# sourmash-bio/sourmash

Measured on AMD Instinct MI355X. Metric: Gbase/s sketched (k=31, scaled=1000), higher is better.
Workload: dtype u64; 1 GPU; C2: sketch synthetic random DNA resident in HBM as ASCII, per GPU 1000 records of 10000000 bases (10000000000 bases, 10000001000 bytes with their separators), k=31 scaled=1000 seed=42; one step = k-mer kernel + radix sort + unique; records_per_gpu=1000, record_len=10000000, bases_per_gpu=10000000000, bytes_per_gpu=10000001000, ksize=31, scaled=1000, unique_hashes_rank0=9998668, unique_hashes_job=9998668, collectives=none (the exchange runs with --full)

## Files before the change

sourmash_amd/csrc/capi_ingest.cpp:

```cpp
#include <stdio.h>
#include <algorithm>
#include <atomic>
#include <chrono>
#include "capi_common.hpp"
#include "ingest.hpp"
#include "pargz.hpp"
#include "residues.hpp"
#include "sigload.hpp"
#include "uniform_sort_core.hpp"

using namespace smg;

namespace {

static size_t sketch_ws_raw_bytes(uint64_t cap) { return al256(cap * 8); }
static size_t sketch_ws_sort_bytes(uint64_t cap, bool counts) {
    return std::max(sort_unique_temp_bytes(cap), sort_unique_uniform_temp_bound(cap, counts));
}

struct SortCounters { std::atomic<uint64_t> bucket{0}, small{0}, fellback{0}; };
static SortCounters& sort_counters() { static SortCounters c; return c; }

static void uniform_sort_and_report(const uint64_t* d_keys, const unsigned long long* d_n, uint64_t n_max, uint64_t thr, uint64_t* d_out,
                                    uint64_t* d_counts, uint64_t* d_n_out, void* d_head, void* d_tmp, size_t tmp_bytes, hipStream_t st,
                                    uint64_t report[3]) {
    uint64_t* d_report = (uint64_t*)d_head;
    uint32_t* d_flag = (uint32_t*)((char*)d_head + 64);
    hip_check(sort_unique_uniform(d_keys, d_n, n_max, thr, d_out, d_counts, d_n_out, d_flag, d_tmp, tmp_bytes, st), "sort_unique_uniform");
    hip_check(sort_report_launch(d_n, d_n_out, d_flag, d_report, st), "sort_report");
    hip_check(hipMemcpyAsync(report, d_report, 24, hipMemcpyDeviceToHost, st), "D2H");
    hip_check(hipStreamSynchronize(st), "sync");
}
static void count_sort_call(uint64_t n_max, uint64_t thr, size_t tmp_bytes, bool counts, bool fellback) {
    if (fellback) ++sort_counters().fellback;
    else if (sort_unique_uniform_form(n_max, thr, tmp_bytes, counts) == US_SMALL) ++sort_counters().small;
    else ++sort_counters().bucket;
}
static int key_bits(uint64_t thr) {
    int bits = 64;
    if (thr != ~0ull) { bits = 1; while (bits < 64 && (thr >> bits)) ++bits; }
    return bits;
}

}

extern "C" {

uint64_t smgpu_signature_add_file(SourmashSignature* p, const char* path, uint64_t* n_records) {
    return landing<uint64_t>([&]() -> uint64_t {
        if (!path) throw err_internal("null path");
        std::vector<KmerMinHash*> mhs;
// ... 107 lines not shown
}

uint64_t smgpu_sketch_dna_raw(const uint8_t* d_seq, uint64_t len, uint32_t ksize, uint64_t seed, uint64_t max_hash,
                              uint64_t* d_out, uint64_t cap, uint64_t* d_result, void* d_ws, uint64_t ws_bytes,
                              void* stream) {
    uint64_t ret = ~0ull;
    landing_void([&] {
        hipStream_t st = (hipStream_t)stream;
        if (ws_bytes < smgpu_sketch_workspace_bytes(cap)) throw err_internal("workspace too small (smgpu_sketch_workspace_bytes)");
        uint64_t* d_raw = (uint64_t*)d_ws;
        void* d_head = (char*)d_ws + sketch_ws_raw_bytes(cap);
        void* d_tmp = (char*)d_head + 256;
        const size_t tmp_bytes = (size_t)(ws_bytes - sketch_ws_raw_bytes(cap) - 256);
        const uint64_t thr = max_hash ? max_hash : ~0ull;
        check_dna_ksize(ksize);
        hip_check(hipMemsetAsync(d_result, 0, 16, st), "memset");
        hip_check(sketch_dna_launch(d_seq, len, ksize, seed, thr, d_raw, (unsigned long long*)d_result, cap, st), "sketch_dna");
        uint64_t report[3] = {0, 0, 0};
        uniform_sort_and_report(d_raw, (const unsigned long long*)d_result, cap, thr, d_out, nullptr, d_result + 1, d_head, d_tmp, tmp_bytes,
                                st, report);
        const uint64_t kept = report[0];
        if (kept > cap)
            throw err_internal("output capacity too small: " + std::to_string(kept) + " kept hashes > capacity " + std::to_string(cap));
        count_sort_call(cap, thr, tmp_bytes, false, report[2] != 0);
        if (report[2] == 0) { ret = report[1]; return; }
        hip_check(sort_unique(d_raw, kept, d_out, nullptr, d_result + 1, d_tmp, tmp_bytes, key_bits(thr), st), "sort_unique");
        unsigned long long nu = 0;
        hip_check(hipMemcpyAsync(&nu, d_result + 1, 8, hipMemcpyDeviceToHost, st), "D2H");
        hip_check(hipStreamSynchronize(st), "sync");
        ret = nu;
    });
    return ret;
}

uint64_t smgpu_sort_unique_uniform_workspace_bytes(uint64_t n_max, int32_t counts) {
// ... 141 lines not shown
```

sourmash_amd/csrc/device_api.hpp:

```cpp
#pragma once
#include <hip/hip_runtime.h>
#include <stdint.h>
#include <stddef.h>
#include "find_core.hpp"

namespace smg {

hipError_t sketch_dna_launch(const uint8_t* d_seq, uint64_t len, uint32_t k, uint64_t seed, uint64_t thr,
                             uint64_t* d_out, unsigned long long* d_count, uint64_t cap, hipStream_t stream);
hipError_t sketch_dna_launch_grid(const uint8_t* d_seq, uint64_t len, uint32_t k, uint64_t seed, uint64_t thr,
                                  uint64_t* d_out, unsigned long long* d_count, uint64_t cap, uint32_t grid, hipStream_t stream);
struct SketchMultiOut { uint64_t thr; uint64_t* out; unsigned long long* count; uint64_t cap; };
bool sketch_dna_multi_supported(const uint32_t* ks, int n);
hipError_t sketch_dna_multi_launch(const uint8_t* d_new, uint64_t n_new, const uint32_t* ks, int n, uint64_t seed, const SketchMultiOut* outs,
                                   hipStream_t stream);
hipError_t sketch_dna_words_launch(const uint8_t* d_seq, uint64_t len, uint32_t k, uint64_t seed, uint64_t thr, uint64_t* d_out,
                                   unsigned long long* d_count, uint64_t cap, bool dense, hipStream_t stream);
uint32_t sketch_dna_max_k();
hipError_t kmer_hashes_launch(const uint8_t* d_seq, uint64_t len, uint32_t k, uint64_t seed, uint64_t* d_out,
                              uint64_t n_kmers, hipStream_t stream);
hipError_t first_invalid_launch(const uint8_t* d_seq, uint64_t len, unsigned long long* d_first, hipStream_t stream);

hipError_t hll_dna_launch(const uint8_t* d_seq, uint64_t len, uint32_t k, uint32_t p, uint32_t* d_regs, hipStream_t stream);
hipError_t hll_hashes_launch(const uint64_t* d_hashes, uint64_t n, uint32_t p, uint32_t* d_regs, bool skip_zero, hipStream_t stream);
// ... 19 lines not shown
hipError_t residue_windows_launch(const uint8_t* d_aa, uint64_t n, uint32_t k, uint64_t seed, uint64_t thr, uint64_t* d_out,
                                  unsigned long long* d_count, uint64_t cap, bool dense, hipStream_t stream);

size_t sort_unique_temp_bytes(uint64_t n);
struct TagSegment { uint64_t src, dst, n; };
hipError_t tag_gather_launch(const uint64_t* d_src, const TagSegment* d_segs, uint32_t n_segs, uint64_t* d_dst, int hbits, hipStream_t stream);
hipError_t sort_unique(uint64_t* d_keys, uint64_t n, uint64_t* d_out, uint64_t* d_counts, uint64_t* d_n_out,
                       void* d_temp, size_t temp_bytes, int bits, hipStream_t stream);

hipError_t sort_unique_uniform(const uint64_t* d_keys, const unsigned long long* d_n, uint64_t n_max, uint64_t thr, uint64_t* d_out,
                               uint64_t* d_counts, uint64_t* d_n_out, uint32_t* d_fellback, void* d_temp, size_t temp_bytes,
                               hipStream_t stream);
size_t sort_unique_uniform_temp_bytes(uint64_t n_max, uint64_t thr, bool counts);
size_t sort_unique_uniform_temp_bound(uint64_t n_max, bool counts);
uint32_t sort_unique_uniform_form(uint64_t n_max, uint64_t thr, size_t temp_bytes, bool counts);
hipError_t sort_report_launch(const unsigned long long* d_n, const uint64_t* d_n_out, const uint32_t* d_fellback, uint64_t* d_report,
                              hipStream_t stream);

size_t sort_pairs_temp_bytes(uint64_t n);
hipError_t sort_pairs(const uint64_t* d_keys_in, uint64_t* d_keys_out, const uint64_t* d_vals_in, uint64_t* d_vals_out, uint64_t n,
                      int bits, void* d_temp, size_t temp_bytes, hipStream_t stream);
size_t rle_pairs_temp_bytes(uint64_t n);
hipError_t rle_pairs(const uint64_t* d_a, const uint64_t* d_b, uint64_t n, uint64_t* d_out_a, uint64_t* d_out_b, uint64_t* d_counts,
                     uint64_t* d_n_out, void* d_temp, size_t temp_bytes, hipStream_t stream);

hipError_t records_pairs_launch(const uint8_t* d_seq, uint64_t len, uint32_t k, uint64_t seed, uint64_t thr, uint64_t* d_hash,
                                uint64_t* d_pos, unsigned long long* d_count, uint64_t cap, hipStream_t stream);
hipError_t records_check_starts_launch(const uint64_t* d_starts, uint64_t n_records, uint64_t len, unsigned long long* d_bad,
                                       hipStream_t stream);
size_t records_csr_temp_bytes(uint64_t n_pairs);
// ... 106 lines not shown
```

sourmash_amd/csrc/kmer_core.hpp:

```cpp
#pragma once
#include "murmur3.hpp"
#include <utility>

namespace smg {

SMG_HD uint32_t perm_b32(uint32_t hi, uint32_t lo, uint32_t sel) {
#if defined(__HIP_DEVICE_COMPILE__)
    return __builtin_amdgcn_perm(hi, lo, sel);
#else
    const uint64_t v = ((uint64_t)hi << 32) | lo;
    uint32_t r = 0;
    for (int i = 0; i < 4; ++i) {
        const uint32_t s = (sel >> (8 * i)) & 0xff;
        uint32_t b;
        if (s < 8) b = (uint32_t)(v >> (8 * s)) & 0xff;
        else if (s == 0x0c) b = 0;
        else b = 0xff;
        r |= b << (8 * i);
    }
    return r;
#endif
}

SMG_HD uint32_t alignbyte_b32(uint32_t hi, uint32_t lo, uint32_t n) {
// ... 229 lines not shown
    process_window<K, P, EARLY, PLAIN, true, LATE>(U, C, dirty, seed, thr, static_cast<Emit&&>(emit), std::make_integer_sequence<int, P>{});
}


template <int K, int P, int BLOCK, int R = 1>
struct TileGeom {
    using G = LaneGeom<K, P>;
    static constexpr int WINDOW = BLOCK * P;
    static constexpr int TILE = R * WINDOW;
    static constexpr int LANE_RD = ((G::NW + 3) / 4) * 4;
    static constexpr int chunks(int rounds) { return ((rounds * BLOCK - 1) * (P / 4) + LANE_RD + 3) / 4; }
    static constexpr int IN_DW = (R * BLOCK - 1) * (P / 4) + LANE_RD;
    static constexpr int IN_CHUNKS = chunks(R);
};

SMG_HD uint32_t sk_tile_rounds(uint64_t thr, uint32_t r_max, uint32_t window, uint32_t cap) {
    if (r_max <= 1) return 1;
    const uint64_t positions = (uint64_t)r_max * window;
    const uint64_t expected = (positions * (thr >> 32)) >> 32;
    return expected + 1 > cap / 4 ? 1u : r_max;
}

SMG_HD uint64_t tile_first(uint32_t workgroup) { return workgroup; }
SMG_HD uint64_t tile_from_ticket(uint32_t grid, uint64_t ticket) { return (uint64_t)grid + ticket; }
SMG_HD bool tile_end(uint64_t tile, uint64_t n_tiles) { return tile >= n_tiles; }

SMG_HD void load_chunk(const uint8_t* seq, uint64_t off, uint64_t len, uint32_t skip, uint32_t* w) {
    w[0] = w[1] = w[2] = w[3] = 0;
    if (off + 16 <= len) {
#if defined(__HIP_DEVICE_COMPILE__)
        const uint4 v = *reinterpret_cast<const uint4*>(seq + off);
        w[0] = v.x; w[1] = v.y; w[2] = v.z; w[3] = v.w;
#else
        for (int b = 0; b < 16; ++b) w[b >> 2] |= (uint32_t)seq[off + b] << (8 * (b & 3));
#endif
// ... 94 lines not shown
        if (cnt < at_least) return;
        const unsigned int n = cnt < (unsigned)CAP ? cnt : (unsigned)CAP;
        if (threadIdx.x == 0) *s_base = atomicAdd(out_count, (unsigned long long)n);
        __syncthreads();
        const unsigned long long b = *s_base;
        for (unsigned int i = threadIdx.x; i < n; i += BLOCK) {
            if (b + i < out_cap) {
#pragma unroll
                for (int j = 0; j < NV; ++j) out[j][b + i] = s_val[j][i];
            }
        }
        __syncthreads();
        if (threadIdx.x == 0) *s_cnt = 0;
    }
};
#endif

}
```

sourmash_amd/csrc/sketch.hip:

```cpp
#include <hip/hip_runtime.h>
#include <stdint.h>
#include <stdlib.h>
#include <utility>
#include "kmer_core.hpp"
#include "sketch_kernel.hpp"
#include "device_api.hpp"

namespace smg {

constexpr int GENERIC_MAX_K = 256;
constexpr int GENERIC_TILE = 4096;

__global__ __launch_bounds__(SK_BLOCK) void sketch_dna_generic_kernel(
    const uint8_t* __restrict__ seq, uint64_t len, uint32_t k, uint64_t seed, uint64_t thr,
    uint64_t* __restrict__ out, unsigned long long* __restrict__ out_count, uint64_t out_cap, uint64_t n_tiles,
    int dense) {
    __shared__ uint8_t s_in[GENERIC_TILE + GENERIC_MAX_K];
    for (uint64_t tile = blockIdx.x; tile < n_tiles; tile += gridDim.x) {
        const uint64_t base = tile * (uint64_t)GENERIC_TILE;
        __syncthreads();
        for (uint32_t i = threadIdx.x; i < GENERIC_TILE + k - 1; i += SK_BLOCK)
            s_in[i] = (base + i < len) ? seq[base + i] : 0;
        __syncthreads();
        for (uint32_t p = threadIdx.x; p < GENERIC_TILE; p += SK_BLOCK) {
// ... 36 lines not shown
    for (uint64_t i = (uint64_t)blockIdx.x * SK_BLOCK + threadIdx.x; i < len; i += (uint64_t)gridDim.x * SK_BLOCK) {
        const uint8_t u = seq[i] & 0xdf;
        if (!(u == 'A' || u == 'C' || u == 'G' || u == 'T')) { best = i; break; }
    }
    if (best != ~0ull) atomicMin(first, best);
}

constexpr int FAST_MAX_K = SK_FAST_MAX_K;
SMG_KMER_PART(SketchLaunch<false>, 0)
SMG_KMER_PART(SketchLaunch<false>, 1)
SMG_KMER_PART(SketchLaunch<false>, 2)
SMG_KMER_PART(SketchLaunch<false>, 3)

static hipError_t sketch_any(const uint8_t* d_seq, uint64_t len, uint32_t k, uint64_t seed, uint64_t thr,
                             uint64_t* d_out, unsigned long long* d_count, uint64_t cap, bool dense,
                             hipStream_t stream, uint32_t grid = 0) {
    if (len < k || k == 0) return hipSuccess;
    static const bool generic_only = [] { const char* e = getenv("SMG_SKETCH_GENERIC"); return e && *e == '1'; }();
    constexpr uint32_t words_from = (uint32_t)FAST_MAX_K + 1u;
    if (k >= words_from && !generic_only) return sketch_dna_words_launch(d_seq, len, k, seed, thr, d_out, d_count, cap, dense, stream);
    if (!dense && k <= (uint32_t)FAST_MAX_K && !generic_only)
        return launcher<SketchLaunch<false>>(k)(d_seq, len, seed, thr, d_out, d_count, cap, grid, stream);
    if (dense && k <= (uint32_t)FAST_MAX_K && !generic_only)
        return launcher<SketchLaunch<true>>(k)(d_seq, len, seed, thr, d_out, d_count, cap, 0, stream);
    if (!generic_only || k > (uint32_t)GENERIC_MAX_K) return sketch_dna_words_launch(d_seq, len, k, seed, thr, d_out, d_count, cap, dense, stream);
    const uint64_t n_tiles = (len + GENERIC_TILE - 1) / GENERIC_TILE;
    hipLaunchKernelGGL(sketch_dna_generic_kernel, dim3(sk_grid(n_tiles)), dim3(SK_BLOCK), 0, stream, d_seq, len, k, seed, thr,
                       d_out, d_count, cap, n_tiles, dense ? 1 : 0);
    return hipGetLastError();
}

hipError_t sketch_dna_launch(const uint8_t* d_seq, uint64_t len, uint32_t k, uint64_t seed, uint64_t thr,
                             uint64_t* d_out, unsigned long long* d_count, uint64_t cap, hipStream_t stream) {
    return sketch_any(d_seq, len, k, seed, thr, d_out, d_count, cap, false, stream);
}

hipError_t sketch_dna_launch_grid(const uint8_t* d_seq, uint64_t len, uint32_t k, uint64_t seed, uint64_t thr,
                                  uint64_t* d_out, unsigned long long* d_count, uint64_t cap, uint32_t grid, hipStream_t stream) {
    return sketch_any(d_seq, len, k, seed, thr, d_out, d_count, cap, false, stream, grid);
}

hipError_t kmer_hashes_launch(const uint8_t* d_seq, uint64_t len, uint32_t k, uint64_t seed, uint64_t* d_out,
                              uint64_t n_kmers, hipStream_t stream) {
    return sketch_any(d_seq, len, k, seed, ~0ull, d_out, nullptr, n_kmers, true, stream);
}

hipError_t first_invalid_launch(const uint8_t* d_seq, uint64_t len, unsigned long long* d_first, hipStream_t stream) {
    if (len == 0) return hipSuccess;
    const uint64_t nb = (len + SK_BLOCK - 1) / SK_BLOCK;
// ... 7 lines not shown
```

sourmash_amd/csrc/sketch_kernel.hpp:

```cpp
#pragma once
#include <hip/hip_runtime.h>
#include <stdint.h>
#include <utility>
#include "kmer_core.hpp"
#include "tile_launch.hpp"
#include "arena.hpp"

namespace smg {

constexpr int SK_BLOCK = 256;
constexpr int SK_FAST_MAX_K = 88;
constexpr int SK_OUT_CAP = 2048;

constexpr bool sk_plain_mul(int k, bool dense) {
    if (dense) return k == 1 || k == 5 || k == 8 || k == 25 || k == 28 || k == 81 || k == 82 || k == 84;
    return k == 50 || k == 51;
}
constexpr bool sk_staged(int k) { return k > 11 && k != 18 && k != 20 && k != 30; }
#ifndef SMG_SK_R_MAX
#define SMG_SK_R_MAX 3
#endif
constexpr int SK_R_MAX = SMG_SK_R_MAX;
static_assert(SK_R_MAX >= 1 && SK_R_MAX <= 3, "four rounds do not fit four workgroups per CU");
constexpr bool sk_late_mask(int k) { return sk_staged(k) && k != 13; }
constexpr bool sk_one_round(int k) { return k <= 17; }
constexpr bool sk_lane16_only(int k) { return (k >= 35 && k <= 40) || (k >= 53 && k <= 56); }
#ifndef SMG_SK_LANE_POSITIONS
#define SMG_SK_LANE_POSITIONS 32
#endif
constexpr int sk_lane_positions(int k, bool dense) {
    return !dense && sk_staged(k) && !sk_one_round(k) && !sk_lane16_only(k) ? SMG_SK_LANE_POSITIONS : 16;
}
#ifndef SMG_SK_LANE32_R_MAX
#define SMG_SK_LANE32_R_MAX 2
#endif
static_assert(SMG_SK_LANE32_R_MAX >= 1 && SMG_SK_LANE32_R_MAX <= 2, "three rounds of 8,192 positions do not fit four workgroups per CU");
constexpr int sk_rounds_max(int k, bool dense) {
    if (dense || !sk_staged(k) || sk_one_round(k)) return 1;
    return sk_lane_positions(k, dense) == 32 ? SMG_SK_LANE32_R_MAX : SK_R_MAX;
// ... 5 lines not shown
#ifdef SMG_SK_STATIC_WALK
constexpr bool sk_handout(int) { return false; }
#else
constexpr bool sk_handout(int) { return true; }
#endif
#ifdef SMG_SK_GRID_PER_CU
constexpr unsigned sk_grid_per_cu(int, bool) { return SMG_SK_GRID_PER_CU; }
#else
constexpr unsigned sk_grid_per_cu(int r_max, bool handout) { return handout ? 0 : r_max > 1 ? 32 : 8; }
#endif

template <int K, int P, bool DENSE>
__global__ __launch_bounds__(SK_BLOCK) void sketch_dna_kernel(
    const uint8_t* __restrict__ seq, uint64_t len, uint64_t seed, uint64_t thr,
    uint64_t* __restrict__ out, unsigned long long* __restrict__ out_count, uint64_t out_cap,
    uint64_t n_tiles, uint32_t skip, uint32_t rounds, unsigned long long* __restrict__ tile_counter) {
    static_assert(P == 16, "the kernel's name; the lane's positions are LP");
    constexpr int LP = sk_lane_positions(K, DENSE);
    constexpr int R_MAX = sk_rounds_max(K, DENSE), OUT_CAP = sk_out_cap(R_MAX, LP);
    using T = TileGeom<K, LP, SK_BLOCK, R_MAX>;
    constexpr int WINDOW = T::WINDOW, LANE_RD = T::LANE_RD, IN_CHUNKS = T::IN_CHUNKS;
    constexpr bool STAGED = !DENSE && sk_staged(K);
    static_assert(R_MAX == 1 || STAGED, "only the staged form walks several rounds");
    const uint32_t n_rounds = R_MAX > 1 ? rounds : 1u;

    __shared__ __attribute__((aligned(16))) uint32_t s_in[IN_CHUNKS * 4];
    __shared__ __attribute__((aligned(16))) uint32_t s_comp[STAGED ? IN_CHUNKS * 4 : 4];
    __shared__ unsigned int s_dirty;
    __shared__ uint64_t s_out[OUT_CAP];
    __shared__ unsigned int s_cnt;
    __shared__ unsigned long long s_base;
    __shared__ unsigned long long s_next;
    const bool handout = !DENSE && sk_handout(K) && tile_counter != nullptr;
    const LdsSink<OUT_CAP, SK_BLOCK> sink{{s_out}, &s_cnt, &s_base, {out}, out_count, out_cap};

    const int tid = threadIdx.x;
    if (tid == 0) s_cnt = 0;

    uint64_t tile = tile_first(blockIdx.x);
    while (!tile_end(tile, n_tiles)) {
        const uint64_t base = tile * ((uint64_t)n_rounds * WINDOW);
        if constexpr (STAGED) {
            if (tid == 0) s_dirty = 0;
        }
        __syncthreads();
        if constexpr (STAGED) {
            if constexpr (R_MAX > 1) stage_tile<IN_CHUNKS, true, SK_BLOCK>(seq, base, len, skip, s_in, s_comp, &s_dirty, T::chunks((int)n_rounds));
            else stage_tile<IN_CHUNKS, true, SK_BLOCK>(seq, base, len, skip, s_in, s_comp, &s_dirty);
        } else {
// ... 52 lines not shown
        __syncthreads();
        if (handout) {
            const unsigned long long next = s_next;
            tile = ((uint64_t)(uint32_t)__builtin_amdgcn_readfirstlane((int)(uint32_t)(next >> 32)) << 32) |
                   (uint32_t)__builtin_amdgcn_readfirstlane((int)(uint32_t)next);
        } else {
            tile += gridDim.x;
        }
        sink.flush(OUT_CAP / 2);
    }
    if constexpr (DENSE) return;
    __syncthreads();
    sink.flush(1);
}

typedef hipError_t (*sketch_launch_fn)(const uint8_t*, uint64_t, uint64_t, uint64_t, uint64_t*, unsigned long long*, uint64_t, uint32_t, hipStream_t);
template <int K, bool DENSE>
unsigned sk_resident_grid() {
    static const unsigned resident = [] {
        int per_cu = 0, dev = 0, cus = 0;
        if (hipOccupancyMaxActiveBlocksPerMultiprocessor(&per_cu, (const void*)sketch_dna_kernel<K, 16, DENSE>, SK_BLOCK, 0) != hipSuccess ||
            hipGetDevice(&dev) != hipSuccess || hipDeviceGetAttribute(&cus, hipDeviceAttributeMultiprocessorCount, dev) != hipSuccess ||
            per_cu < 1 || cus < 1) {
            (void)hipGetLastError();
            return 2048u;
        }
        return (unsigned)per_cu * (unsigned)cus;
    }();
    return resident;
}
template <bool DENSE>
struct SketchLaunch {
    using fn = sketch_launch_fn;
    static constexpr int KMAX = SK_FAST_MAX_K;
    template <int K>
    static hipError_t launch(const uint8_t* d_seq, uint64_t len, uint64_t seed, uint64_t thr, uint64_t* d_out,
                             unsigned long long* d_count, uint64_t cap, uint32_t grid, hipStream_t stream) {
        constexpr uint32_t LP = (uint32_t)sk_lane_positions(K, DENSE), WINDOW = (uint32_t)SK_BLOCK * LP;
        constexpr uint32_t R_MAX = (uint32_t)sk_rounds_max(K, DENSE);
        const uint32_t rounds = sk_tile_rounds(thr, R_MAX, WINDOW, (uint32_t)sk_out_cap((int)R_MAX, (int)LP));
        const TileSpan t = align_to_tiles(d_seq, len, (uint64_t)rounds * WINDOW);
        if (t.n_tiles == 0) return hipSuccess;
        constexpr unsigned per_cu = sk_grid_per_cu((int)R_MAX, !DENSE && sk_handout(K));
        unsigned g;
        if (grid && !DENSE) {
            g = grid;
        } else if constexpr (per_cu == 0) {
            const unsigned resident = sk_resident_grid<K, DENSE>();
            g = (unsigned)(t.n_tiles < resident ? t.n_tiles : resident);
        } else {
            g = sk_grid(t.n_tiles, per_cu);
        }
        ArenaBuf counter;
        if constexpr (!DENSE && sk_handout(K)) {
            if (t.n_tiles > g) {
                hipError_t e = counter.get(8, stream);
                if (e == hipSuccess) e = hipMemsetAsync(counter.p, 0, 8, stream);
                if (e != hipSuccess) return e;
            }
        }
        hipLaunchKernelGGL((sketch_dna_kernel<K, 16, DENSE>), dim3(g), dim3(SK_BLOCK), 0, stream,
                           t.seq, t.len, seed, thr, d_out, d_count, cap, t.n_tiles, t.skip, rounds, counter.as<unsigned long long>());
        return hipGetLastError();
    }
};

}
```

sourmash_amd/csrc/uniform_sort.hip:

```cpp
#include <hip/hip_runtime.h>
#include "device_api.hpp"
#include "uniform_sort_core.hpp"

namespace smg {
namespace {

constexpr uint32_t NO_BASE = 0xffffffffu;

__device__ __forceinline__ uint64_t us_count(const unsigned long long* d_n, uint64_t n_max) {
    const uint64_t n = *d_n;
    return n < n_max ? n : n_max;
}

template <int T>
__device__ __forceinline__ void us_sort_lds(uint64_t* keys, uint32_t n) {
    const uint32_t P = us_pow2(n);
    for (uint32_t k = 2, j = 0; k <= P; us_next_step(k, j)) {
        for (uint32_t t = threadIdx.x; t < P / 2; t += T) {
            uint32_t a, b;
            us_pair(t, k, j, a, b);
            us_compare_exchange(keys, n, a, b);
        }
        __syncthreads();
    }
// ... 212 lines not shown
    __shared__ uint32_t bins[US_LEAF_BINS + 1];
    __shared__ uint32_t scan[256 / 64];
    if (*d_fellback) return;
    const uint64_t leaf = blockIdx.x;
    const uint32_t held = cursor[leaf];
    const uint32_t n = held < US_LEAF_CAP ? held : US_LEAF_CAP;
    uint64_t* mine = leaves + leaf * US_LEAF_CAP;
    us_sort_keys<256, US_LEAF_CAP / 256, US_LEAF_BINS, true>(mine, n, shift, s, bins, scan);
    const uint32_t total = us_unique_write<256, US_LEAF_CAP / 256, uint32_t>(s, n, scan, mine,
                                                                            leaf_counts ? leaf_counts + leaf * US_LEAF_CAP : nullptr);
    if (threadIdx.x == 0) leaf_distinct[leaf] = total;
}

__global__ __launch_bounds__(1024) void us_scan_kernel(const uint32_t* __restrict__ leaf_distinct, uint32_t n_leaves,
                                                       uint32_t* __restrict__ offsets, uint64_t* __restrict__ d_n_out,
                                                       const uint32_t* __restrict__ d_fellback) {
    __shared__ uint32_t wsum[1024 / 64];
    if (*d_fellback) return;
    uint32_t carry = 0;
    for (uint32_t base = 0; base < n_leaves; base += 4096) {
        const uint32_t l = base + threadIdx.x * 4;
        uint32_t v[4], sum = 0, total;
#pragma unroll
        for (int i = 0; i < 4; ++i) {
            v[i] = l + i < n_leaves ? leaf_distinct[l + i] : 0;
            sum += v[i];
        }
        uint32_t at = carry + us_block_scan<1024>(sum, wsum, total);
#pragma unroll
        for (int i = 0; i < 4; ++i) {
            if (l + i < n_leaves) offsets[l + i] = at;
            at += v[i];
        }
        carry += total;
    }
    if (threadIdx.x == 0) {
        offsets[n_leaves] = carry;
        *d_n_out = carry;
    }
}

__global__ __launch_bounds__(256) void us_pack_kernel(const uint64_t* __restrict__ leaves, const uint32_t* __restrict__ leaf_counts,
                                                      const uint32_t* __restrict__ offsets, uint64_t* __restrict__ out,
                                                      uint64_t* __restrict__ counts, const uint32_t* __restrict__ d_fellback) {
    if (*d_fellback) return;
    const uint64_t leaf = blockIdx.x;
    const uint32_t at = offsets[leaf], n = offsets[leaf + 1] - at;
    for (uint32_t i = threadIdx.x; i < n; i += 256) {
        out[at + i] = leaves[leaf * US_LEAF_CAP + i];
        if (counts) counts[at + i] = leaf_counts[leaf * US_LEAF_CAP + i];
    }
}

// ... 12 lines not shown
UsLayout us_layout(const UsPlan& p, bool counts) {
    UsLayout y{};
    const size_t n_leaf_cursors = p.form == US_TWO_PASS ? (size_t)p.regions * US_FANOUT : US_FANOUT;
    y.coarse_cursors = 0;
    y.leaf_cursors = up256(US_FANOUT * 4);
    y.cursor_bytes = y.leaf_cursors + up256(n_leaf_cursors * 4);
    y.distinct = y.cursor_bytes;
    y.offsets = y.distinct + up256(n_leaf_cursors * 4);
    y.coarse = y.offsets + up256((n_leaf_cursors + 1) * 4);
    y.leaves = y.coarse + up256((size_t)p.regions * p.region_cap * 8);
    y.counts = y.leaves + up256((size_t)p.leaves * US_LEAF_CAP * 8);
    y.total = y.counts + (counts ? up256((size_t)p.leaves * US_LEAF_CAP * 4) : 0);
    return y;
}

}

size_t sort_unique_uniform_temp_bytes(uint64_t n_max, uint64_t thr, bool counts) {
    const UsPlan p = us_plan(n_max, thr);
    if (p.form == US_SMALL || p.form == US_DECLINE) return 256;
    return us_layout(p, counts).total;
}

size_t sort_unique_uniform_temp_bound(uint64_t n_max, bool counts) {
    if (n_max <= US_SMALL_MAX) return 256;
    return up256((size_t)n_max * 8 * 5 + (counts ? (size_t)n_max * 4 * 3 : 0) + ((size_t)8 << 20));
}

uint32_t sort_unique_uniform_form(uint64_t n_max, uint64_t thr, size_t temp_bytes, bool counts) {
    const UsPlan p = us_plan(n_max, thr);
    if (p.form == US_SMALL || p.form == US_DECLINE) return p.form;
    return temp_bytes < us_layout(p, counts).total ? (uint32_t)US_DECLINE : p.form;
}

hipError_t sort_unique_uniform(const uint64_t* d_keys, const unsigned long long* d_n, uint64_t n_max, uint64_t thr, uint64_t* d_out,
                               uint64_t* d_counts, uint64_t* d_n_out, uint32_t* d_fellback, void* d_temp, size_t temp_bytes,
                               hipStream_t stream) {
    const UsPlan p = us_plan(n_max, thr);
    const uint32_t form = sort_unique_uniform_form(n_max, thr, temp_bytes, d_counts != nullptr);
    if (form == US_SMALL) {
        hipLaunchKernelGGL(us_small_kernel, dim3(1), dim3(1024), 0, stream, d_keys, d_n, n_max, us_small_shift(thr), d_out, d_counts, d_n_out,
                           d_fellback);
        return hipGetLastError();
    }
    if (form == US_DECLINE) return hipMemsetD32Async((hipDeviceptr_t)d_fellback, 1, 1, stream);
    const UsLayout y = us_layout(p, d_counts != nullptr);
    char* base = (char*)d_temp;
    uint32_t* coarse_cursors = (uint32_t*)(base + y.coarse_cursors);
    uint32_t* leaf_cursors = (uint32_t*)(base + y.leaf_cursors);
    uint32_t* distinct = (uint32_t*)(base + y.distinct);
    uint32_t* offsets = (uint32_t*)(base + y.offsets);
    uint64_t* coarse = (uint64_t*)(base + y.coarse);
    uint64_t* leaves = (uint64_t*)(base + y.leaves);
    uint32_t* leaf_counts = d_counts ? (uint32_t*)(base + y.counts) : nullptr;
    hipError_t e = hipMemsetAsync(d_fellback, 0, 4, stream);
    if (e != hipSuccess) return e;
    e = hipMemsetAsync(base, 0, y.cursor_bytes, stream);
    if (e != hipSuccess) return e;
    const uint32_t tiles = (uint32_t)((n_max + US_TILE - 1) / US_TILE);
    if (form == US_ONE_PASS) {
        hipLaunchKernelGGL(us_scatter_kernel<false>, dim3(tiles), dim3(256), 0, stream, p, d_keys, d_n, n_max, (const uint32_t*)nullptr, 1u,
                           leaf_cursors, leaves, (uint64_t)US_LEAF_CAP, d_fellback);
    } else {
        hipLaunchKernelGGL(us_scatter_kernel<false>, dim3(tiles), dim3(256), 0, stream, p, d_keys, d_n, n_max, (const uint32_t*)nullptr, 1u,
                           coarse_cursors, coarse, p.region_cap, d_fellback);
        const uint32_t tpr = (uint32_t)((p.region_cap + US_TILE - 1) / US_TILE);
        hipLaunchKernelGGL(us_scatter_kernel<true>, dim3((uint32_t)p.regions * tpr), dim3(256), 0, stream, p, (const uint64_t*)coarse, d_n,
                           n_max, (const uint32_t*)coarse_cursors, tpr, leaf_cursors, leaves, (uint64_t)US_LEAF_CAP, d_fellback);
    }
    const uint32_t L = (uint32_t)p.leaves;
    hipLaunchKernelGGL(us_leaf_kernel, dim3(L), dim3(256), 0, stream, p.shift, (const uint32_t*)leaf_cursors, leaves, leaf_counts, distinct,
                       (const uint32_t*)d_fellback);
    hipLaunchKernelGGL(us_scan_kernel, dim3(1), dim3(1024), 0, stream, (const uint32_t*)distinct, L, offsets, d_n_out,
                       (const uint32_t*)d_fellback);
    hipLaunchKernelGGL(us_pack_kernel, dim3(L), dim3(256), 0, stream, (const uint64_t*)leaves, (const uint32_t*)leaf_counts,
                       (const uint32_t*)offsets, d_out, d_counts, (const uint32_t*)d_fellback);
    return hipGetLastError();
}

hipError_t sort_report_launch(const unsigned long long* d_n, const uint64_t* d_n_out, const uint32_t* d_fellback, uint64_t* d_report,
                              hipStream_t stream) {
    hipLaunchKernelGGL(us_report_kernel, dim3(1), dim3(1), 0, stream, d_n, d_n_out, d_fellback, d_report);
    return hipGetLastError();
}

}
```

sourmash_amd/csrc/uniform_sort_core.hpp:

```cpp
#pragma once
#include <stdint.h>

#if defined(__HIPCC__)
#include <hip/hip_runtime.h>
#endif

#ifndef SMG_HD
#if defined(__HIPCC__)
#define SMG_HD __host__ __device__ __forceinline__
#else
#define SMG_HD inline
#endif
#endif

namespace smg {

constexpr uint32_t US_SMALL_MAX = 16384;
constexpr uint32_t US_LEAF_CAP = 1024;
constexpr uint32_t US_FANOUT = 256;
constexpr uint32_t US_TILE = 4096;
constexpr uint64_t US_MAX_LEAVES = (uint64_t)US_FANOUT * US_FANOUT;

enum UsForm : uint32_t { US_DECLINE = 0, US_SMALL = 1, US_ONE_PASS = 2, US_TWO_PASS = 3 };

// ... 42 lines not shown
}

SMG_HD uint64_t us_leaf_of(const UsPlan& p, uint64_t key) { return key >> p.shift; }
SMG_HD uint32_t us_digit_first(const UsPlan& p, uint64_t key) {
    if (key > p.thr) return US_FANOUT;
    const uint64_t leaf = us_leaf_of(p, key);
    return (uint32_t)(p.form == US_TWO_PASS ? leaf >> 8 : leaf);
}
SMG_HD uint32_t us_digit_second(const UsPlan& p, uint64_t region, uint64_t key) {
    if (key > p.thr) return US_FANOUT;
    const uint64_t leaf = us_leaf_of(p, key);
    return (leaf >> 8) == region ? (uint32_t)(leaf & 0xff) : US_FANOUT;
}
SMG_HD bool us_reserve_ok(uint64_t base, uint64_t count, uint64_t cap) { return base <= cap && count <= cap - base; }

constexpr uint32_t US_LEAF_BINS = 1024;
constexpr uint32_t US_SMALL_BINS = 4096;
constexpr uint32_t US_BIN_LIMIT = 32;
SMG_HD uint32_t us_bin_leaf(uint32_t shift, uint64_t key) { return (uint32_t)(key >> (shift > 10 ? shift - 10 : 0)) & (US_LEAF_BINS - 1); }
SMG_HD uint32_t us_small_shift(uint64_t thr) {
    uint32_t s = 0;
    while (s < 63 && (thr >> s) >= US_SMALL_BINS) ++s;
    return s;
}
SMG_HD uint32_t us_bin_small(uint32_t small_shift, uint64_t key) {
    const uint64_t b = key >> small_shift;
    return b < US_SMALL_BINS ? (uint32_t)b : US_SMALL_BINS - 1;
}
SMG_HD bool us_before(uint64_t other, uint32_t other_at, uint64_t key, uint32_t at) { return other < key || (other == key && other_at < at); }

// ... 25 lines not shown
```

Before: 384.5 Gbase/s.

## Scatter sketch hashes directly into uniform-sort leaf buckets from the k-mer kernel

The sketch kernel's LDS sink now also reserves a slot per hash in the uniform sort's leaf buckets via atomic cursors and stores the key there, so the sort only runs the leaf/scan/pack stages. This removes the separate scatter kernel(s) and a re-read of the raw hash array, and merges the report into the scan kernel. In exchange the flush does extra global atomics per kept hash and still writes the raw array for fallback.

```diff
diff --git a/sourmash_amd/csrc/capi_ingest.cpp b/sourmash_amd/csrc/capi_ingest.cpp
--- a/sourmash_amd/csrc/capi_ingest.cpp
+++ b/sourmash_amd/csrc/capi_ingest.cpp
@@ -1,4 +1,5 @@
 #include <stdio.h>
+#include <stdlib.h>
 #include <algorithm>
 #include <atomic>
 #include <chrono>
@@ -35,6 +36,10 @@
     if (fellback) ++sort_counters().fellback;
     else if (sort_unique_uniform_form(n_max, thr, tmp_bytes, counts) == US_SMALL) ++sort_counters().small;
     else ++sort_counters().bucket;
+}
+static bool leaf_sink_enabled() {
+    const char* e = getenv("SMG_SKETCH_LEAF_SINK");
+    return !(e && e[0] == '0' && e[1] == 0);
 }
 static int key_bits(uint64_t thr) {
     int bits = 64;
@@ -172,11 +177,22 @@
         const size_t tmp_bytes = (size_t)(ws_bytes - sketch_ws_raw_bytes(cap) - 256);
         const uint64_t thr = max_hash ? max_hash : ~0ull;
         check_dna_ksize(ksize);
+        uint32_t* d_flag = (uint32_t*)((char*)d_head + 64);
+        UsLeafTarget target{};
+        if (leaf_sink_enabled()) hip_check(sort_unique_uniform_begin(cap, thr, d_flag, d_tmp, tmp_bytes, st, &target), "sort_unique_uniform_begin");
         hip_check(hipMemsetAsync(d_result, 0, 16, st), "memset");
-        hip_check(sketch_dna_launch(d_seq, len, ksize, seed, thr, d_raw, (unsigned long long*)d_result, cap, st), "sketch_dna");
+        bool fed = false;
+        hip_check(sketch_dna_launch(d_seq, len, ksize, seed, thr, d_raw, (unsigned long long*)d_result, cap, st, &target, &fed), "sketch_dna");
         uint64_t report[3] = {0, 0, 0};
-        uniform_sort_and_report(d_raw, (const unsigned long long*)d_result, cap, thr, d_out, nullptr, d_result + 1, d_head, d_tmp, tmp_bytes,
-                                st, report);
+        if (fed) {
+            hip_check(sort_unique_uniform_finish((const unsigned long long*)d_result, cap, thr, d_out, d_result + 1, d_flag, d_tmp, tmp_bytes,
+                                                 (uint64_t*)d_head, st), "sort_unique_uniform_finish");
+            hip_check(hipMemcpyAsync(report, d_head, 24, hipMemcpyDeviceToHost, st), "D2H");
+            hip_check(hipStreamSynchronize(st), "sync");
+        } else {
+            uniform_sort_and_report(d_raw, (const unsigned long long*)d_result, cap, thr, d_out, nullptr, d_result + 1, d_head, d_tmp, tmp_bytes,
+                                    st, report);
+        }
         const uint64_t kept = report[0];
         if (kept > cap)
             throw err_internal("output capacity too small: " + std::to_string(kept) + " kept hashes > capacity " + std::to_string(cap));
diff --git a/sourmash_amd/csrc/device_api.hpp b/sourmash_amd/csrc/device_api.hpp
--- a/sourmash_amd/csrc/device_api.hpp
+++ b/sourmash_amd/csrc/device_api.hpp
@@ -3,11 +3,13 @@
 #include <stdint.h>
 #include <stddef.h>
 #include "find_core.hpp"
+#include "uniform_sort_core.hpp"
 
 namespace smg {
 
 hipError_t sketch_dna_launch(const uint8_t* d_seq, uint64_t len, uint32_t k, uint64_t seed, uint64_t thr,
-                             uint64_t* d_out, unsigned long long* d_count, uint64_t cap, hipStream_t stream);
+                             uint64_t* d_out, unsigned long long* d_count, uint64_t cap, hipStream_t stream,
+                             const UsLeafTarget* leaf = nullptr, bool* fed = nullptr);
 hipError_t sketch_dna_launch_grid(const uint8_t* d_seq, uint64_t len, uint32_t k, uint64_t seed, uint64_t thr,
                                   uint64_t* d_out, unsigned long long* d_count, uint64_t cap, uint32_t grid, hipStream_t stream);
 struct SketchMultiOut { uint64_t thr; uint64_t* out; unsigned long long* count; uint64_t cap; };
@@ -57,6 +59,10 @@
 size_t sort_unique_uniform_temp_bytes(uint64_t n_max, uint64_t thr, bool counts);
 size_t sort_unique_uniform_temp_bound(uint64_t n_max, bool counts);
 uint32_t sort_unique_uniform_form(uint64_t n_max, uint64_t thr, size_t temp_bytes, bool counts);
+hipError_t sort_unique_uniform_begin(uint64_t n_max, uint64_t thr, uint32_t* d_fellback, void* d_temp, size_t temp_bytes, hipStream_t stream,
+                                     UsLeafTarget* target);
+hipError_t sort_unique_uniform_finish(const unsigned long long* d_n, uint64_t n_max, uint64_t thr, uint64_t* d_out, uint64_t* d_n_out,
+                                      uint32_t* d_fellback, void* d_temp, size_t temp_bytes, uint64_t* d_report, hipStream_t stream);
 hipError_t sort_report_launch(const unsigned long long* d_n, const uint64_t* d_n_out, const uint32_t* d_fellback, uint64_t* d_report,
                               hipStream_t stream);
 
diff --git a/sourmash_amd/csrc/kmer_core.hpp b/sourmash_amd/csrc/kmer_core.hpp
--- a/sourmash_amd/csrc/kmer_core.hpp
+++ b/sourmash_amd/csrc/kmer_core.hpp
@@ -1,5 +1,6 @@
 #pragma once
 #include "murmur3.hpp"
+#include "uniform_sort_core.hpp"
 #include <utility>
 
 namespace smg {
@@ -267,11 +268,13 @@
     static constexpr int IN_CHUNKS = chunks(R);
 };
 
+SMG_HD bool sk_tile_sparse(uint64_t thr, uint64_t positions, uint32_t cap) {
+    const uint64_t expected = (positions * (thr >> 32)) >> 32;
+    return expected + 1 <= cap / 4;
+}
 SMG_HD uint32_t sk_tile_rounds(uint64_t thr, uint32_t r_max, uint32_t window, uint32_t cap) {
     if (r_max <= 1) return 1;
-    const uint64_t positions = (uint64_t)r_max * window;
-    const uint64_t expected = (positions * (thr >> 32)) >> 32;
-    return expected + 1 > cap / 4 ? 1u : r_max;
+    return sk_tile_sparse(thr, (uint64_t)r_max * window, cap) ? r_max : 1u;
 }
 
 SMG_HD uint64_t tile_first(uint32_t workgroup) { return workgroup; }
@@ -396,6 +399,46 @@
         if (threadIdx.x == 0) *s_cnt = 0;
     }
 };
-#endif
-
-}
+
+template <int CAP, int BLOCK>
+struct LeafSink : LdsSink<CAP, BLOCK, 1> {
+    UsLeafTarget leaf;
+
+    __device__ __forceinline__ void flush(unsigned int at_least) const {
+        if (!us_has_target(leaf)) { LdsSink<CAP, BLOCK, 1>::flush(at_least); return; }
+        static_assert(CAP % BLOCK == 0, "entries per lane");
+        constexpr int E = CAP / BLOCK;
+        const unsigned int cnt = *this->s_cnt;
+        if (cnt < at_least) return;
+        const unsigned int n = cnt < (unsigned)CAP ? cnt : (unsigned)CAP;
+        uint64_t v[E];
+        uint32_t slot[E];
+#pragma unroll
+        for (int e = 0; e < E; ++e) {
+            const unsigned int i = threadIdx.x + (unsigned)e * BLOCK;
+            if (i < n) {
+                v[e] = this->s_val[0][i];
+                slot[e] = us_leaf_slot(leaf, v[e]);
+            }
+        }
+        if (threadIdx.x == 0) {
+            if (cnt > (unsigned)CAP) us_raise(leaf.fellback);
+            *this->s_base = atomicAdd(this->out_count, (unsigned long long)n);
+        }
+        __syncthreads();
+        const unsigned long long b = *this->s_base;
+#pragma unroll
+        for (int e = 0; e < E; ++e) {
+            const unsigned int i = threadIdx.x + (unsigned)e * BLOCK;
+            if (i < n) {
+                if (b + i < this->out_cap) this->out[0][b + i] = v[e];
+                us_leaf_store(leaf, v[e], slot[e]);
+            }
+        }
+        __syncthreads();
+        if (threadIdx.x == 0) *this->s_cnt = 0;
+    }
+};
+#endif
+
+}
diff --git a/sourmash_amd/csrc/sketch.hip b/sourmash_amd/csrc/sketch.hip
--- a/sourmash_amd/csrc/sketch.hip
+++ b/sourmash_amd/csrc/sketch.hip
@@ -74,15 +74,16 @@
 
 static hipError_t sketch_any(const uint8_t* d_seq, uint64_t len, uint32_t k, uint64_t seed, uint64_t thr,
                              uint64_t* d_out, unsigned long long* d_count, uint64_t cap, bool dense,
-                             hipStream_t stream, uint32_t grid = 0) {
+                             hipStream_t stream, uint32_t grid = 0, const UsLeafTarget* leaf = nullptr, bool* fed = nullptr) {
+    if (fed) *fed = false;
     if (len < k || k == 0) return hipSuccess;
     static const bool generic_only = [] { const char* e = getenv("SMG_SKETCH_GENERIC"); return e && *e == '1'; }();
     constexpr uint32_t words_from = (uint32_t)FAST_MAX_K + 1u;
     if (k >= words_from && !generic_only) return sketch_dna_words_launch(d_seq, len, k, seed, thr, d_out, d_count, cap, dense, stream);
     if (!dense && k <= (uint32_t)FAST_MAX_K && !generic_only)
-        return launcher<SketchLaunch<false>>(k)(d_seq, len, seed, thr, d_out, d_count, cap, grid, stream);
+        return launcher<SketchLaunch<false>>(k)(d_seq, len, seed, thr, d_out, d_count, cap, grid, stream, leaf, fed);
     if (dense && k <= (uint32_t)FAST_MAX_K && !generic_only)
-        return launcher<SketchLaunch<true>>(k)(d_seq, len, seed, thr, d_out, d_count, cap, 0, stream);
+        return launcher<SketchLaunch<true>>(k)(d_seq, len, seed, thr, d_out, d_count, cap, 0, stream, nullptr, nullptr);
     if (!generic_only || k > (uint32_t)GENERIC_MAX_K) return sketch_dna_words_launch(d_seq, len, k, seed, thr, d_out, d_count, cap, dense, stream);
     const uint64_t n_tiles = (len + GENERIC_TILE - 1) / GENERIC_TILE;
     hipLaunchKernelGGL(sketch_dna_generic_kernel, dim3(sk_grid(n_tiles)), dim3(SK_BLOCK), 0, stream, d_seq, len, k, seed, thr,
@@ -91,8 +92,9 @@
 }
 
 hipError_t sketch_dna_launch(const uint8_t* d_seq, uint64_t len, uint32_t k, uint64_t seed, uint64_t thr,
-                             uint64_t* d_out, unsigned long long* d_count, uint64_t cap, hipStream_t stream) {
-    return sketch_any(d_seq, len, k, seed, thr, d_out, d_count, cap, false, stream);
+                             uint64_t* d_out, unsigned long long* d_count, uint64_t cap, hipStream_t stream, const UsLeafTarget* leaf,
+                             bool* fed) {
+    return sketch_any(d_seq, len, k, seed, thr, d_out, d_count, cap, false, stream, 0, leaf, fed);
 }
 
 hipError_t sketch_dna_launch_grid(const uint8_t* d_seq, uint64_t len, uint32_t k, uint64_t seed, uint64_t thr,
diff --git a/sourmash_amd/csrc/sketch_kernel.hpp b/sourmash_amd/csrc/sketch_kernel.hpp
--- a/sourmash_amd/csrc/sketch_kernel.hpp
+++ b/sourmash_amd/csrc/sketch_kernel.hpp
@@ -1,6 +1,7 @@
 #pragma once
 #include <hip/hip_runtime.h>
 #include <stdint.h>
+#include <type_traits>
 #include <utility>
 #include "kmer_core.hpp"
 #include "tile_launch.hpp"
@@ -23,6 +24,7 @@
 constexpr int SK_R_MAX = SMG_SK_R_MAX;
 static_assert(SK_R_MAX >= 1 && SK_R_MAX <= 3, "four rounds do not fit four workgroups per CU");
 constexpr bool sk_late_mask(int k) { return sk_staged(k) && k != 13; }
+constexpr bool sk_leaf_sink(int k) { return k <= 33 && k != 20 && k != 24 && k != 28 && k != 32; }
 constexpr bool sk_one_round(int k) { return k <= 17; }
 constexpr bool sk_lane16_only(int k) { return (k >= 35 && k <= 40) || (k >= 53 && k <= 56); }
 #ifndef SMG_SK_LANE_POSITIONS
@@ -58,7 +60,7 @@
 __global__ __launch_bounds__(SK_BLOCK) void sketch_dna_kernel(
     const uint8_t* __restrict__ seq, uint64_t len, uint64_t seed, uint64_t thr,
     uint64_t* __restrict__ out, unsigned long long* __restrict__ out_count, uint64_t out_cap,
-    uint64_t n_tiles, uint32_t skip, uint32_t rounds, unsigned long long* __restrict__ tile_counter) {
+    uint64_t n_tiles, uint32_t skip, uint32_t rounds, unsigned long long* __restrict__ tile_counter, const UsLeafTarget leaf) {
     static_assert(P == 16, "the kernel's name; the lane's positions are LP");
     constexpr int LP = sk_lane_positions(K, DENSE);
     constexpr int R_MAX = sk_rounds_max(K, DENSE), OUT_CAP = sk_out_cap(R_MAX, LP);
@@ -76,7 +78,12 @@
     __shared__ unsigned long long s_base;
     __shared__ unsigned long long s_next;
     const bool handout = !DENSE && sk_handout(K) && tile_counter != nullptr;
-    const LdsSink<OUT_CAP, SK_BLOCK> sink{{s_out}, &s_cnt, &s_base, {out}, out_count, out_cap};
+    constexpr bool LEAVES = !DENSE && sk_leaf_sink(K);
+    const LdsSink<OUT_CAP, SK_BLOCK> plain_sink{{s_out}, &s_cnt, &s_base, {out}, out_count, out_cap};
+    const typename std::conditional<LEAVES, LeafSink<OUT_CAP, SK_BLOCK>, LdsSink<OUT_CAP, SK_BLOCK>>::type sink = [&] {
+        if constexpr (LEAVES) return LeafSink<OUT_CAP, SK_BLOCK>{plain_sink, leaf};
+        else return plain_sink;
+    }();
 
     const int tid = threadIdx.x;
     if (tid == 0) s_cnt = 0;
@@ -159,7 +166,8 @@
     sink.flush(1);
 }
 
-typedef hipError_t (*sketch_launch_fn)(const uint8_t*, uint64_t, uint64_t, uint64_t, uint64_t*, unsigned long long*, uint64_t, uint32_t, hipStream_t);
+typedef hipError_t (*sketch_launch_fn)(const uint8_t*, uint64_t, uint64_t, uint64_t, uint64_t*, unsigned long long*, uint64_t, uint32_t, hipStream_t,
+                                       const UsLeafTarget*, bool*);
 template <int K, bool DENSE>
 unsigned sk_resident_grid() {
     static const unsigned resident = [] {
@@ -180,12 +188,18 @@
     static constexpr int KMAX = SK_FAST_MAX_K;
     template <int K>
     static hipError_t launch(const uint8_t* d_seq, uint64_t len, uint64_t seed, uint64_t thr, uint64_t* d_out,
-                             unsigned long long* d_count, uint64_t cap, uint32_t grid, hipStream_t stream) {
+                             unsigned long long* d_count, uint64_t cap, uint32_t grid, hipStream_t stream, const UsLeafTarget* leaf,
+                             bool* fed) {
         constexpr uint32_t LP = (uint32_t)sk_lane_positions(K, DENSE), WINDOW = (uint32_t)SK_BLOCK * LP;
         constexpr uint32_t R_MAX = (uint32_t)sk_rounds_max(K, DENSE);
         const uint32_t rounds = sk_tile_rounds(thr, R_MAX, WINDOW, (uint32_t)sk_out_cap((int)R_MAX, (int)LP));
         const TileSpan t = align_to_tiles(d_seq, len, (uint64_t)rounds * WINDOW);
         if (t.n_tiles == 0) return hipSuccess;
+        UsLeafTarget target{};
+        if constexpr (!DENSE && sk_leaf_sink(K)) {
+            if (leaf && us_has_target(*leaf) && sk_tile_sparse(thr, (uint64_t)R_MAX * WINDOW,(uint32_t)sk_out_cap((int)R_MAX, (int)LP))) target = *leaf;
+        }
+        if (fed) *fed = us_has_target(target);
         constexpr unsigned per_cu = sk_grid_per_cu((int)R_MAX, !DENSE && sk_handout(K));
         unsigned g;
         if (grid && !DENSE) {
@@ -205,7 +219,7 @@
             }
         }
         hipLaunchKernelGGL((sketch_dna_kernel<K, 16, DENSE>), dim3(g), dim3(SK_BLOCK), 0, stream,
-                           t.seq, t.len, seed, thr, d_out, d_count, cap, t.n_tiles, t.skip, rounds, counter.as<unsigned long long>());
+                           t.seq, t.len, seed, thr, d_out, d_count, cap, t.n_tiles, t.skip, rounds, counter.as<unsigned long long>(), target);
         return hipGetLastError();
     }
 };
diff --git a/sourmash_amd/csrc/uniform_sort.hip b/sourmash_amd/csrc/uniform_sort.hip
--- a/sourmash_amd/csrc/uniform_sort.hip
+++ b/sourmash_amd/csrc/uniform_sort.hip
@@ -250,9 +250,17 @@
 
 __global__ __launch_bounds__(1024) void us_scan_kernel(const uint32_t* __restrict__ leaf_distinct, uint32_t n_leaves,
                                                        uint32_t* __restrict__ offsets, uint64_t* __restrict__ d_n_out,
-                                                       const uint32_t* __restrict__ d_fellback) {
+                                                       const uint32_t* __restrict__ d_fellback, const unsigned long long* __restrict__ d_n,
+                                                       uint64_t* __restrict__ report) {
     __shared__ uint32_t wsum[1024 / 64];
-    if (*d_fellback) return;
+    if (*d_fellback) {
+        if (report && threadIdx.x == 0) {
+            report[0] = *d_n;
+            report[1] = *d_n_out;
+            report[2] = 1;
+        }
+        return;
+    }
     uint32_t carry = 0;
     for (uint32_t base = 0; base < n_leaves; base += 4096) {
         const uint32_t l = base + threadIdx.x * 4;
@@ -273,6 +281,11 @@
     if (threadIdx.x == 0) {
         offsets[n_leaves] = carry;
         *d_n_out = carry;
+        if (report) {
+            report[0] = *d_n;
+            report[1] = carry;
+            report[2] = 0;
+        }
     }
 }
 
@@ -315,6 +328,30 @@
     return y;
 }
 
+struct UsRegions {
+    uint32_t *coarse_cursors, *leaf_cursors, *distinct, *offsets;
+    uint64_t *coarse, *leaves;
+    uint32_t* leaf_counts;
+    size_t cursor_bytes;
+};
+UsRegions us_regions(const UsLayout& y, void* d_temp, bool counts) {
+    char* base = (char*)d_temp;
+    return {(uint32_t*)(base + y.coarse_cursors), (uint32_t*)(base + y.leaf_cursors), (uint32_t*)(base + y.distinct), (uint32_t*)(base + y.offsets),
+            (uint64_t*)(base + y.coarse), (uint64_t*)(base + y.leaves), counts ? (uint32_t*)(base + y.counts) : nullptr, y.cursor_bytes};
+}
+
+hipError_t us_leaves_finish(const UsPlan& p, const UsRegions& r, const unsigned long long* d_n, uint64_t* d_out, uint64_t* d_counts,
+                            uint64_t* d_n_out, uint32_t* d_fellback, uint64_t* d_report, hipStream_t stream) {
+    const uint32_t L = (uint32_t)p.leaves;
+    hipLaunchKernelGGL(us_leaf_kernel, dim3(L), dim3(256), 0, stream, p.shift, (const uint32_t*)r.leaf_cursors, r.leaves, r.leaf_counts, r.distinct,
+                       (const uint32_t*)d_fellback);
+    hipLaunchKernelGGL(us_scan_kernel, dim3(1), dim3(1024), 0, stream, (const uint32_t*)r.distinct, L, r.offsets, d_n_out,
+                       (const uint32_t*)d_fellback, d_n, d_report);
+    hipLaunchKernelGGL(us_pack_kernel, dim3(L), dim3(256), 0, stream, (const uint64_t*)r.leaves, (const uint32_t*)r.leaf_counts,
+                       (const uint32_t*)r.offsets, d_out, d_counts, (const uint32_t*)d_fellback);
+    return hipGetLastError();
+}
+
 }
 
 size_t sort_unique_uniform_temp_bytes(uint64_t n_max, uint64_t thr, bool counts) {
@@ -345,38 +382,53 @@
         return hipGetLastError();
     }
     if (form == US_DECLINE) return hipMemsetD32Async((hipDeviceptr_t)d_fellback, 1, 1, stream);
-    const UsLayout y = us_layout(p, d_counts != nullptr);
-    char* base = (char*)d_temp;
-    uint32_t* coarse_cursors = (uint32_t*)(base + y.coarse_cursors);
-    uint32_t* leaf_cursors = (uint32_t*)(base + y.leaf_cursors);
-    uint32_t* distinct = (uint32_t*)(base + y.distinct);
-    uint32_t* offsets = (uint32_t*)(base + y.offsets);
-    uint64_t* coarse = (uint64_t*)(base + y.coarse);
-    uint64_t* leaves = (uint64_t*)(base + y.leaves);
-    uint32_t* leaf_counts = d_counts ? (uint32_t*)(base + y.counts) : nullptr;
+    const UsRegions r = us_regions(us_layout(p, d_counts != nullptr), d_temp, d_counts != nullptr);
     hipError_t e = hipMemsetAsync(d_fellback, 0, 4, stream);
     if (e != hipSuccess) return e;
-    e = hipMemsetAsync(base, 0, y.cursor_bytes, stream);
+    e = hipMemsetAsync(d_temp, 0, r.cursor_bytes, stream);
     if (e != hipSuccess) return e;
     const uint32_t tiles = (uint32_t)((n_max + US_TILE - 1) / US_TILE);
     if (form == US_ONE_PASS) {
         hipLaunchKernelGGL(us_scatter_kernel<false>, dim3(tiles), dim3(256), 0, stream, p, d_keys, d_n, n_max, (const uint32_t*)nullptr, 1u,
-                           leaf_cursors, leaves, (uint64_t)US_LEAF_CAP, d_fellback);
+                           r.leaf_cursors, r.leaves, (uint64_t)US_LEAF_CAP, d_fellback);
     } else {
         hipLaunchKernelGGL(us_scatter_kernel<false>, dim3(tiles), dim3(256), 0, stream, p, d_keys, d_n, n_max, (const uint32_t*)nullptr, 1u,
-                           coarse_cursors, coarse, p.region_cap, d_fellback);
+                           r.coarse_cursors, r.coarse, p.region_cap, d_fellback);
         const uint32_t tpr = (uint32_t)((p.region_cap + US_TILE - 1) / US_TILE);
-        hipLaunchKernelGGL(us_scatter_kernel<true>, dim3((uint32_t)p.regions * tpr), dim3(256), 0, stream, p, (const uint64_t*)coarse, d_n,
-                           n_max, (const uint32_t*)coarse_cursors, tpr, leaf_cursors, leaves, (uint64_t)US_LEAF_CAP, d_fellback);
-    }
-    const uint32_t L = (uint32_t)p.leaves;
-    hipLaunchKernelGGL(us_leaf_kernel, dim3(L), dim3(256), 0, stream, p.shift, (const uint32_t*)leaf_cursors, leaves, leaf_counts, distinct,
-                       (const uint32_t*)d_fellback);
-    hipLaunchKernelGGL(us_scan_kernel, dim3(1), dim3(1024), 0, stream, (const uint32_t*)distinct, L, offsets, d_n_out,
-                       (const uint32_t*)d_fellback);
-    hipLaunchKernelGGL(us_pack_kernel, dim3(L), dim3(256), 0, stream, (const uint64_t*)leaves, (const uint32_t*)leaf_counts,
-                       (const uint32_t*)offsets, d_out, d_counts, (const uint32_t*)d_fellback);
-    return hipGetLastError();
+        hipLaunchKernelGGL(us_scatter_kernel<true>, dim3((uint32_t)p.regions * tpr), dim3(256), 0, stream, p, (const uint64_t*)r.coarse, d_n,
+                           n_max, (const uint32_t*)r.coarse_cursors, tpr, r.leaf_cursors, r.leaves, (uint64_t)US_LEAF_CAP, d_fellback);
+    }
+    return us_leaves_finish(p, r, nullptr, d_out, d_counts, d_n_out, d_fellback, nullptr, stream);
+}
+
+hipError_t sort_unique_uniform_begin(uint64_t n_max, uint64_t thr, uint32_t* d_fellback, void* d_temp, size_t temp_bytes, hipStream_t stream,
+                                     UsLeafTarget* target) {
+    *target = UsLeafTarget{};
+    const uint32_t form = sort_unique_uniform_form(n_max, thr, temp_bytes, false);
+    if (form == US_SMALL || form == US_DECLINE) return hipSuccess;
+    const UsPlan p = us_plan(n_max, thr);
+    const UsLayout y = us_layout(p, false);
+    const UsRegions r = us_regions(y, d_temp, false);
+    char* const flag = (char*)d_fellback;
+    char* const cursors_end = (char*)d_temp + y.cursor_bytes;
+    hipError_t e;
+    if (flag < (char*)d_temp && (char*)d_temp - flag <= 4096) {
+        e = hipMemsetAsync(flag, 0, (size_t)(cursors_end - flag), stream);
+    } else {
+        e = hipMemsetAsync(d_fellback, 0, 4, stream);
+        if (e == hipSuccess) e = hipMemsetAsync(r.leaf_cursors, 0, y.cursor_bytes - y.leaf_cursors, stream);
+    }
+    if (e != hipSuccess) return e;
+    *target = UsLeafTarget{r.leaf_cursors, r.leaves, d_fellback, p.shift, (uint32_t)p.leaves};
+    return hipSuccess;
+}
+
+hipError_t sort_unique_uniform_finish(const unsigned long long* d_n, uint64_t n_max, uint64_t thr, uint64_t* d_out, uint64_t* d_n_out,
+                                      uint32_t* d_fellback, void* d_temp, size_t temp_bytes, uint64_t* d_report, hipStream_t stream) {
+    const uint32_t form = sort_unique_uniform_form(n_max, thr, temp_bytes, false);
+    if (form == US_SMALL || form == US_DECLINE) return hipErrorInvalidValue;
+    const UsPlan p = us_plan(n_max, thr);
+    return us_leaves_finish(p, us_regions(us_layout(p, false), d_temp, false), d_n, d_out, nullptr, d_n_out, d_fellback, d_report, stream);
 }
 
 hipError_t sort_report_launch(const unsigned long long* d_n, const uint64_t* d_n_out, const uint32_t* d_fellback, uint64_t* d_report,
diff --git a/sourmash_amd/csrc/uniform_sort_core.hpp b/sourmash_amd/csrc/uniform_sort_core.hpp
--- a/sourmash_amd/csrc/uniform_sort_core.hpp
+++ b/sourmash_amd/csrc/uniform_sort_core.hpp
@@ -80,6 +80,42 @@
 }
 SMG_HD bool us_reserve_ok(uint64_t base, uint64_t count, uint64_t cap) { return base <= cap && count <= cap - base; }
 
+struct UsLeafTarget {
+    uint32_t* cursor;
+    uint64_t* leaves;
+    uint32_t* fellback;
+    uint32_t shift;
+    uint32_t n_leaves;
+};
+SMG_HD bool us_has_target(const UsLeafTarget& t) { return t.cursor != nullptr; }
+SMG_HD uint32_t us_fetch_add(uint32_t* p, uint32_t v) {
+#if defined(__HIP_DEVICE_COMPILE__)
+    return atomicAdd(p, v);
+#else
+    const uint32_t old = *p;
+    *p = old + v;
+    return old;
+#endif
+}
+SMG_HD void us_raise(uint32_t* flag) {
+#if defined(__HIP_DEVICE_COMPILE__)
+    atomicOr(flag, 1u);
+#else
+    *flag |= 1u;
+#endif
+}
+constexpr uint32_t US_NO_SLOT = 0xffffffffu;
+SMG_HD uint32_t us_leaf_slot(const UsLeafTarget& t, uint64_t key) {
+    const uint64_t leaf = key >> t.shift;
+    if (leaf >= t.n_leaves) { us_raise(t.fellback); return US_NO_SLOT; }
+    return us_fetch_add(&t.cursor[leaf], 1u);
+}
+SMG_HD void us_leaf_store(const UsLeafTarget& t, uint64_t key, uint32_t slot) {
+    if (slot < US_LEAF_CAP) t.leaves[(key >> t.shift) * US_LEAF_CAP + slot] = key;
+    else if (slot != US_NO_SLOT) us_raise(t.fellback);
+}
+SMG_HD void us_leaf_put(const UsLeafTarget& t, uint64_t key) { us_leaf_store(t, key, us_leaf_slot(t, key)); }
+
 constexpr uint32_t US_LEAF_BINS = 1024;
 constexpr uint32_t US_SMALL_BINS = 4096;
 constexpr uint32_t US_BIN_LIMIT = 32;
```

Result: no change. 388.2 Gbase/s (median of 6 runs) (+1.0%).
